# DYZhang09/ToC3D

Measured on AMD Instinct MI355X. Metric: multi-view frames/sec through ViT+ToC3D backbone, 6x(800x320), higher is better.
Workload: dtype bf16; 1 GPU; toc3d_faster EVA-02 ViT-L backbone + CPFPN neck, 6 views x 3x320x800 per frame, 1 frame per rank per step, random-init weights, prev_exists=True, injected Gumbel noise; frames_per_forward=1, launch=recorded launch plan replayed from C (toc3d_plan_run, HIP streams), view_groups=1, alias_outputs=True, gather_bytes=0

## Files before the change

include/toc3d.h:

```cpp
#ifndef TOC3D_H_
#define TOC3D_H_

#include <stdint.h>

#ifdef __cplusplus
extern "C" {
#endif

#define TOC3D_ABI_VERSION 10

#define TOC3D_OK 0
#define TOC3D_ERR_ARG (-1)
#define TOC3D_ERR_UNSUPPORTED (-2)
#define TOC3D_ERR_LAUNCH (-3)

#define TOC3D_DTYPE_F32 0
#define TOC3D_DTYPE_BF16 1
#define TOC3D_DTYPE_F32X3 2
#define TOC3D_DTYPE_F32X6 3
#define TOC3D_DTYPE_F32X3W 4
#define TOC3D_DTYPE_F32X3P 5
#define TOC3D_DTYPE_F32X3WO 6
#define TOC3D_DTYPE_F32X3WA 7

#define TOC3D_EPI_BIAS 0
#define TOC3D_EPI_RESIDUAL 1
#define TOC3D_EPI_SWIGLU 2
#define TOC3D_EPI_GELU 3
#define TOC3D_EPI_SWIGLU_STATS 4
#define TOC3D_EPI_RESIDUAL_LN 5
#define TOC3D_EPI_RESIDUAL_STATS 6
#define TOC3D_EPI_SWIGLU_STATS_LN 7
// ... 89 lines not shown
                               const int32_t* count, const int32_t* count_k, const int32_t* npad, const void* pad_rot, int64_t stride,
                               int64_t nwin, int64_t max_count, int64_t num_heads, const float* v_bias,
                               int64_t n_prefetch, const void* const* prefetch_ptrs, const int64_t* prefetch_bytes, int64_t prefetch_workgroups,
                               toc3d_stream_t stream);

int toc3d_gather_merge_ln(int dtype, const float* x, int64_t C, const int32_t* tok, const float* wgt, const int32_t* crow_tok,
                          const int32_t* rep_row, int64_t nW, int64_t N, int64_t k, int64_t rows, const float* gamma,
                          const float* beta, float eps, float* shortcut, void* a_out, int64_t lda, toc3d_stream_t stream);
int toc3d_gather_merge_ln_ex(int dtype, const float* x, int64_t C, const int32_t* tok, const float* wgt, const int32_t* crow_tok,
                             const int32_t* rep_row, int64_t nW, int64_t N, int64_t k, int64_t rows, const float* gamma,
                             const float* beta, float eps, float* shortcut, void* a_out, int64_t lda, int64_t kept_copy, toc3d_stream_t stream);
#define TOC3D_GATHER_SPLIT_COUNTER_BYTES 16384
int64_t toc3d_gather_merge_ln_scratch_bytes(int64_t nW, int64_t C);
int toc3d_gather_merge_ln_split(int dtype, const float* x, int64_t C, const int32_t* tok, const float* wgt, const int32_t* crow_tok,
                                const int32_t* rep_row, int64_t nW, int64_t N, int64_t k, int64_t rows, const float* gamma,
                                const float* beta, float eps, float* shortcut, void* a_out, int64_t lda, int64_t kept_copy,
                                void* scratch, int64_t scratch_bytes, int64_t split, toc3d_stream_t stream);
int toc3d_rebase_layernorm_rows(int dtype, float* slow, int64_t C, const int32_t* rep_index, const int32_t* tok, const float* wgt, int64_t N,
                                int64_t k, const float* rep_raw1, const float* rep_raw2, const float* gamma, const float* beta, float eps,
                                void* out, int64_t ldo, int64_t rows, toc3d_stream_t stream);
int toc3d_scatter_update(float* x, int64_t C, const int32_t* tok, const int32_t* prow, int64_t nW, int64_t N, int64_t k,
                         const float* slow_out, const float* rep_raw1, const float* rep_raw2, const float* rep_raw3, const float* rep_raw4,
                         toc3d_stream_t stream);

int64_t toc3d_motion_weights_floats(void);
int toc3d_pack_motion_weights(const float* qe0_w, const float* qe0_b, const float* qe2_w, const float* qe2_b,
                              const float* pe_red_w, const float* pe_red_b, const float* pe_gam_w, const float* pe_gam_b,
                              const float* pe_bet_w, const float* pe_bet_b, const float* q_red_w, const float* q_red_b,
                              const float* q_gam_w, const float* q_gam_b, const float* q_bet_w, const float* q_bet_b,
                              const float* te_w, const float* te_b, const float* te_ln_w, const float* te_ln_b,
                              const float* pc_range, const float* dimt3, const float* dimt1, float* out,
                              toc3d_stream_t stream);
int toc3d_motion_queries(const float* w, int64_t n_stages, int64_t w_stride, const float* queries, const float* ref_points,
                         const float* vel, const void* timestamp, int timestamp_is_f64, const float* ego_pose,
                         const float* ego_pose_inv, int64_t B, int64_t Q, float* out, toc3d_stream_t stream);
int toc3d_collapse_query_scorer(const float* mq, const float* w_in, const float* b_in, const float* w_agg, const float* b_agg,
                                int64_t B, int64_t Q, int64_t C, float scale, float* wc, float* bc, toc3d_stream_t stream);
int toc3d_score_tokens(const float* x, int64_t C, const float* mask, const float* wc, const float* bc, const float* gumbel,
                       int64_t V, int64_t T, int64_t views_per_frame, float* pred, float* score, float* mask_out,
                       toc3d_stream_t stream);

int toc3d_gumbel_noise(float* out, int64_t n, uint64_t seed, uint64_t* state, toc3d_stream_t stream);
int toc3d_gumbel_from_bits(const uint32_t* bits, int64_t n, float* out, toc3d_stream_t stream);

int toc3d_global_mean_half(int dtype, void* t, int64_t ld, int64_t V, int64_t T, int64_t C, toc3d_stream_t stream);
int toc3d_score_head(int dtype, const void* f, int64_t ld, int64_t kdim, const float* w, const float* b, const float* gumbel,
// ... 68 lines not shown
```

toc3d_amd/backbone.py:

```python
from __future__ import annotations

import math
from functools import partial
from typing import Dict

import torch
import torch.nn as nn

from . import gemm, lib
from .gemm import DEFAULT_PRECISION, round_up
from .plan import MODES, DerivedState, EagerExec, run_frame
from .synth import MOTION_DIM, QUERY_DIM, rope_tables


class ToC3DViTReturnType:

    def __init__(self, img_feats=None, token_masks=None, attn_scores=None, keep_idx=None, drop_idx=None,
                 aux_outputs: list = None) -> None:
        self.img_feats = img_feats
        self.token_masks = token_masks
        self.attn_scores = attn_scores
        self.keep_idx = keep_idx
        self.drop_idx = drop_idx
        self.aux_outputs = aux_outputs
# ... 92 lines not shown
            nn.init.constant_(m.bias, 0)
    elif isinstance(m, nn.LayerNorm):
        nn.init.constant_(m.bias, 0)
        nn.init.constant_(m.weight, 1.0)


def schedule_defaults(precision):
    bf16 = precision == "bf16"
    fast = precision in ("bf16", "fp32x3")
    return dict(
        x3_attention=precision == "fp32x3",
        x3_planes=precision == "fp32x3",
        carry_compact=fast,
        fold_ffn_ln=fast,
        fold_norm2=fast,
        gathered_residual=True,
        prefetch_weights=192 if bf16 else 0,
        attn_rot=fast,
        gather_split=False,
        side_lanes=True,
        big_windows_first=True,
        launch_mode="plan",
    )


class _BackboneBase(DerivedState, nn.Module):
    LN_EPS = 1e-6
    SCORER_LN_EPS = 1e-5

    def _setup_common(self, img_size, patch_size, in_chans, embed_dim, depth, num_heads, mlp_ratio, qkv_bias,
                      use_abs_pos, pt_hw_seq_len, window_size, global_window_size, global_attn_indexes,
                      pretrain_img_size, pretrain_use_cls_token, out_feature, precision, img_norm_cfg=None, pad_size_divisor=32, schedule=None):
        assert precision in ("bf16", "fp32", "fp32x3", "fp32x6"), precision
        self.img_norm_cfg = None
        if img_norm_cfg is not None:
            self.img_norm_cfg = dict(mean=torch.tensor(list(img_norm_cfg["mean"]), dtype=torch.float32),
                                     std=torch.tensor(list(img_norm_cfg["std"]), dtype=torch.float32),
                                     to_rgb=bool(img_norm_cfg.get("to_rgb", True)))
            assert self.img_norm_cfg["mean"].numel() == 3 and self.img_norm_cfg["std"].numel() == 3
        self.pad_size_divisor = int(pad_size_divisor)
        assert self.pad_size_divisor % patch_size == 0, "PadMultiViewImage divisor must be a multiple of the patch size"
        if embed_dim // num_heads != 64 or embed_dim % num_heads:
            raise NotImplementedError("the HIP attention kernel is built for head_dim 64 (EVA-02 L/B/tiny test config)")
        if embed_dim % 64 or embed_dim > 1024:
            raise NotImplementedError("embed_dim must be a multiple of 64 and <= 1024")
        self.precision = precision
# ... 3 lines not shown
        self.global_attn_indexes = tuple(global_attn_indexes)
        self.pretrain_use_cls_token = pretrain_use_cls_token
        self.hidden_dim = int(embed_dim * mlp_ratio)
        self.patch_embed = _PatchEmbed(in_chans, embed_dim, patch_size)
        if use_abs_pos:
            npatch = (pretrain_img_size // patch_size) ** 2
            self.pos_embed = nn.Parameter(torch.zeros(1, npatch + (1 if pretrain_use_cls_token else 0), embed_dim))
        else:
            self.pos_embed = None
        half = embed_dim // num_heads // 2
        self.rope_win = _Rope(window_size, half, pt_hw_seq_len)
        self.rope_glb = _Rope(img_size // patch_size, half, pt_hw_seq_len)
        if img_size // patch_size != global_window_size:
            raise NotImplementedError("global RoPE table side (img_size/patch) must equal global_window_size")
        self._out_features = [out_feature]
        self._out_feature_channels = {out_feature: embed_dim}
        self._out_feature_strides = {out_feature: patch_size}
        self._drop_derived()
        self._tuned: Dict[tuple, int] = {}
        self.autotune = True
        self.alias_outputs = False
        self.view_groups = 1
        sched = schedule_defaults(precision)
        unknown = set(schedule or {}) - set(sched)
        if unknown:
            raise TypeError(f"unknown schedule switches {sorted(unknown)}; known: {sorted(sched)}")
        sched.update(schedule or {})
        for k_, v_ in sched.items():
            setattr(self, k_, v_)
        assert self.launch_mode in MODES, self.launch_mode
        self._stream_pool = []

    _DERIVED = dict(_packed=None, _plans={}, _sk_ws={}, _sk_ws_old=[])
    _INSTANCE = dict(_stream_pool=[])

    def __getstate__(self):
        d = super().__getstate__()
        if d.get("_gumbel_rng") is not None:
            d["_gumbel_rng"] = d["_gumbel_rng"].detach().to("cpu").clone()
        return d

    def __setstate__(self, d):
        if "gumbel_seed" in d and "_gumbel_seed" not in d:
            d = dict(d)
            d["_gumbel_seed"] = d.pop("gumbel_seed")
        super().__setstate__(d)

    def _accelerated(self, i):
        return False

    @property
    def _dts(self):
        return gemm.dtypes(self.precision, self.x3_planes, self.x3_attention)

    _dt = property(lambda self: self._dts.act)
    _tdt = property(lambda self: self._dts.torch)
    _dt_gemm = property(lambda self: self._dts.gemm)
    _dt_rows = property(lambda self: self._dts.rows)
    _dt_attn = property(lambda self: self._dts.attn)
    _x3p = property(lambda self: self._dts.x3p)

    def _block_side(self, i):
        return self.global_window_size if i in self.global_attn_indexes else self.window_size

    @staticmethod
    def _f32(t):
        return t.detach().float().contiguous()

# ... 160 lines not shown
    def _stem_im2col(self, plan, img):
        s = lib.stream_ptr()
        V = plan["V"]
        H, W = plan["h"] * self.patch_size, plan["w"] * self.patch_size
        Kp = plan["col"].shape[1]
        if img.dtype == torch.uint8:
            n = self.img_norm_cfg
            lib.call("toc3d_im2col_patches_u8", self._dt, img, V, img.shape[1], img.shape[2], n["mean"], n["std"], int(n["to_rgb"]),
                     plan["col"], Kp, H, W, self.patch_size, s)
        else:
            lib.call("toc3d_im2col_patches", self._dt, img, plan["col"], Kp, V, self.in_chans, H, W, self.patch_size, s)

    def _stem_gemm(self, plan, P):
        C = self.embed_dim
        pos = P["pos"][(plan["h"], plan["w"])]
        self._linear(lib.EPI_RESIDUAL, plan["col"], P["w_patch"], P["b_patch"], plan["x"], plan["M"], C, plan["col"].shape[1],
                     residual=pos, ldr=C, residual_row_mod=plan["T"] if pos is not None else 0)

    def _ensure_pos(self, P, h, w, dev):
        if (h, w) not in P["pos"]:
            P["pos"][(h, w)] = self._pos_for(h, w, dev)

    def _run_frame(self, master, n_lanes, frame_fn, variant=None):
        run_frame(master.setdefault("launch", {}).setdefault(variant, {}), self.launch_mode, n_lanes, frame_fn, self._stream_pool)

    def _attention(self, P, i, *args):
        s = lib.stream_ptr()
        if not self.prefetch_weights:
            lib.call("toc3d_window_attention", *args, s)
            return
        lib.call("toc3d_window_attention_pf", *args, *self._prefetch_args(P, i), s)

    def _prefetch_args(self, P, i):
        bp = P["blocks"][i]
        ts = [bp["wproj"], bp["w12"], bp["w3"]] + ([P["blocks"][i + 1]["wqkv"]] if i + 1 < self.depth else [])
        if not self.prefetch_weights:
            ts = []
        return (len(ts), *lib.ptr_arrays(ts, min_len=1), self.prefetch_weights)

    def _qkv_attention(self, P, i, plan, M, rope_rc, arows, aslots, count_q, count_k, npad, pad, stride, nwin, max_count, v_bias):
        bp = P["blocks"][i]
        C, dt = self.embed_dim, self._dt
        if self._rot_ok(stride):
            self._linear(lib.EPI_QKV_ROPE, plan["a"], bp["wqkv"], bp["bqkv"], plan["qkv"], M, 3 * C, C,
                         rope=(rope_rc, bp["rope_tab"], bp["rope_side"], lib.ATTN_ROT_Q_SCALE), a_planes=self._x3p, o_planes=self._x3p)
            if self._x3p:
                lib.call("toc3d_window_attention_rot", lib.F32X3P, plan["qkv"], 3 * C, plan["att"], C, arows, aslots, count_q, count_k, npad, pad, stride, nwin, max_count,
# ... 3 lines not shown
                     self.num_heads, v_bias, *self._prefetch_args(P, i), lib.stream_ptr())
            return
        self._linear(lib.EPI_BIAS, plan["a"], bp["wqkv"], bp["bqkv"], plan["qkv"], M, 3 * C, C, a_planes=self._x3p)
        self._attention(P, i, self._dt_attn, plan["qkv"], 3 * C, plan["att"], C, arows, aslots, count_q, count_k, npad, pad,
                        stride, nwin, max_count, self.num_heads, bp["cos"], bp["sin"], bp["rope_side"], v_bias, 64 ** -0.5)

    def _rot_ok(self, stride):
        if not self.attn_rot:
            return False
        if self.precision == "bf16":
            return stride <= 416
        return self._x3p and stride <= 1024

    def _proj(self, bp, plan, rows, out, rep_out, rep_index, res=None, res_index=None):
        C = self.embed_dim
        res = out if res is None else res
        kw = dict(residual=res, ldr=C, rep_out=rep_out, rep_index=rep_index, residual_index=res_index, a_planes=self._x3p)
        if self.fold_norm2:
            self._linear(lib.EPI_RESIDUAL_STATS, plan["att"], bp["wproj"], bp["bproj"], out, rows, C, C, stats_out=(plan["stats2"], plan["stats2_cap"]),
                         out_act=plan["a"], ld_act=C, o_planes=self._x3p, **kw)
        else:
            self._linear(lib.EPI_RESIDUAL, plan["att"], bp["wproj"], bp["bproj"], out, rows, C, C, **kw)

    def _mlp(self, bp, plan, rows, res, rep_out, rep_index):
        s = lib.stream_ptr()
        C, Hd = self.embed_dim, self.hidden_dim
        Hp = plan["hid"].shape[1]
        dt = self._dt
        if self.fold_ffn_ln:
            st, cap = plan["stats"], plan["stats_cap"]
            if self.fold_norm2:
                self._linear(lib.EPI_SWIGLU_STATS_LN, plan["a"], bp["w12"], bp["c2_12"], plan["hid"], rows, 2 * Hp, C, n_valid=Hd, stats_out=(st, cap),
                             stats_in=(plan["stats2"], plan["stats2_cap"], C // 64), col_sums=bp["c1_12"], ln_n=C, ln_eps=self.LN_EPS,
                             a_planes=self._x3p, o_planes=self._x3p)
            else:
                lib.call("toc3d_layernorm_rows", dt, res, C, None, None, bp["ln2_w"], bp["ln2_b"], self.LN_EPS, plan["a"], C, rows, C, s)
                self._linear(lib.EPI_SWIGLU_STATS, plan["a"], bp["w12"], bp["b12"], plan["hid"], rows, 2 * Hp, C, n_valid=Hd, stats_out=(st, cap), o_planes=self._x3p)
            self._linear(lib.EPI_RESIDUAL_LN, plan["hid"], bp["w3"], bp["c2"], res, rows, C, Hp, residual=res, ldr=C, rep_out=rep_out, rep_index=rep_index,
                         stats_in=(st, cap, -(-2 * Hp // 128)), col_sums=bp["c1"], ln_n=Hd, ln_eps=self.LN_EPS, a_planes=self._x3p)
            return
        lib.call("toc3d_layernorm_rows", dt, res, C, None, None, bp["ln2_w"], bp["ln2_b"], self.LN_EPS, plan["a"], C, rows, C, s)
        self._linear(lib.EPI_SWIGLU, plan["a"], bp["w12"], bp["b12"], plan["hid"], rows, 2 * Hp, C, n_valid=Hd)
        lib.call("toc3d_layernorm_act", dt, plan["hid"], Hp, bp["lnf_w"], bp["lnf_b"], self.LN_EPS, plan["hln"], Hp, rows, Hd, s)
        self._linear(lib.EPI_RESIDUAL, plan["hln"], bp["w3"], bp["b3"], res, rows, C, Hp, residual=res, ldr=C, rep_out=rep_out, rep_index=rep_index)

    def _dense_block(self, i, plan, P):
        s = lib.stream_ptr()
        bp = P["blocks"][i]
        C, M, dt = self.embed_dim, plan["M"], self._dt
        x = plan["x"]
        dm = plan["dense"][self._block_side(i)]
        lib.call("toc3d_layernorm_rows", self._dt_rows, x, C, None, None, bp["ln1_w"], bp["ln1_b"], self.LN_EPS, plan["a"], C, M, C, s)
        self._qkv_attention(P, i, plan, M, dm.get("rc"), dm["rows"], dm["slots"], dm["count"], None, dm["npad"], None, dm["N"], dm["nW"], dm["max_count"], bp["v_bias"])
        self._proj(bp, plan, M, x, None, None)
        self._mlp(bp, plan, M, x, None, None)

    def _group_layout(self, V, B):
        G = max(1, int(self.view_groups))
        vpf = V // B
        if G > 1 and V % G == 0:
            Vg = V // G
            if Vg % vpf == 0:
                return [(g * Vg, Vg, g * (Vg // vpf), Vg // vpf) for g in range(G)]
            if vpf % Vg == 0:
                return [(g * Vg, Vg, (g * Vg) // vpf, 1) for g in range(G)]
        return [(0, V, 0, B)]

# ... 376 lines not shown
            self._join_side(ex, lane, side, plan)
            plan["side_L"] = None
        sel = plan["sel"][(st, self._block_side(i))]
        nW, N, k, rows = sel["nW"], sel["N"], sel["k"], sel["rows"]
        slow = plan["slow"]
        if carry_in:
            lib.call("toc3d_rebase_layernorm_rows", self._dt_rows, slow, C, sel["rep_index"], sel["tok"], sel["wgt"], N, k, plan["rep1"], plan["rep2"],
                     bp["ln1_w"], bp["ln1_b"], self.LN_EPS, plan["a"], C, rows, s)
        elif self.gather_split:
            lib.call("toc3d_gather_merge_ln_split", self._dt_rows, plan["x"], C, sel["tok"], sel["wgt"], sel["crow_tok"], sel["rep_row"], nW, N, k, rows,
                     bp["ln1_w"], bp["ln1_b"], self.LN_EPS, slow, plan["a"], C, 0 if self.gathered_residual else 1,
                     plan["gm_scratch"], plan["gm_scratch"].numel() * 4, int(self.gather_split) if self.gather_split is not True else 0, s)
        else:
            lib.call("toc3d_gather_merge_ln_ex", self._dt_rows, plan["x"], C, sel["tok"], sel["wgt"], sel["crow_tok"], sel["rep_row"], nW, N, k, rows,
                     bp["ln1_w"], bp["ln1_b"], self.LN_EPS, slow, plan["a"], C, 0 if self.gathered_residual else 1, s)
        rot = self._rot_ok(k + 1)
        self._qkv_attention(P, i, plan, rows, sel["crow_rc"], sel["arows"], sel["aslots"], sel["acount_q"], sel["acount_k"], None,
                            bp["pad_rot"] if rot else bp["pad_qkv"], k + 1, nW, sel["max_q"], None)
        ra, rb = (plan["rep3"], plan["rep4"]) if carry_in else (plan["rep1"], plan["rep2"])
        if self.gathered_residual and not carry_in:
            self._proj(bp, plan, rows, slow, ra, sel["rep_index"], res=plan["x"], res_index=sel["crow_tok"])
        else:
            self._proj(bp, plan, rows, slow, ra, sel["rep_index"])
        self._mlp(bp, plan, rows, slow, rb, sel["rep_index"])
        if not carry_out:
            lib.call("toc3d_scatter_update", plan["x"], C, sel["tok"], sel["prow"], nW, N, k, slow, plan["rep1"], plan["rep2"],
                     plan["rep3"] if carry_in else None, plan["rep4"] if carry_in else None, s)

    def _carries(self, i):
        return (self.carry_compact and i + 1 < self.depth and self._accelerated(i) and self._accelerated(i + 1)
                and (i + 1) not in self.pruning_loc and self._block_side(i) == self._block_side(i + 1))

    @torch.no_grad()
    def forward(self, x, temp_queries=None, prev_exists=None, temp_ref_points=None, temp_vel=None, temp_timestamp=None,
                temp_ego_pose=None, ego_pose_inv=None, *args, gumbel_noise=None, **kwargs):
        if "forced_scores" in kwargs:
            raise TypeError("forced_scores is a test instrument: wrap the model with toc3d_amd.testing.instrument(model)")
        x, H, W = self._check_input(x)
        if self._packed is None:
            self._packed = self._pack()
            self._plans = {}
        P = self._packed
        dev = x.device
        V = x.shape[0]
        prev = bool(prev_exists.bool().flatten()[0].item()) if isinstance(prev_exists, torch.Tensor) else bool(prev_exists)
        B = temp_queries.shape[0] if temp_queries is not None else 1
        assert V % B == 0
        ns = len(self.pruning_loc)
        key = (tuple(x.shape), x.dtype, B, self.view_groups)
        if key in self._plans:
# ... 103 lines not shown
```

toc3d_amd/csrc/gemm.hip:

```cpp
#include <cstdlib>

#include "gemm_kernels.h"

thread_local bool g_bad_variant = false;

namespace {

int launch_gemm(int is_bf16, int epi, int variant, const GemmArgs& a, hipStream_t s) {
    switch (epi) {
        case TOC3D_EPI_BIAS: case TOC3D_EPI_GELU: case TOC3D_EPI_CONV3X3: return toc3d_gemm_launch_plain(is_bf16, epi, variant, a, s);
        case TOC3D_EPI_RESIDUAL: case TOC3D_EPI_RESIDUAL_LN: case TOC3D_EPI_RESIDUAL_STATS: return toc3d_gemm_launch_residual(is_bf16, epi, variant, a, s);
        case TOC3D_EPI_SWIGLU: case TOC3D_EPI_SWIGLU_STATS: case TOC3D_EPI_SWIGLU_STATS_LN: return toc3d_gemm_launch_swiglu(is_bf16, epi, variant, a, s);
        case TOC3D_EPI_QKV_ROPE: return toc3d_gemm_launch_rope(is_bf16, epi, variant, a, s);
        default: return TOC3D_ERR_ARG;
    }
}

__global__ __launch_bounds__(256) void x3_planes_kernel(const float* src, int64_t ld_src, float* dst, int64_t ld_dst, int64_t rows, int gpr) {
    const int64_t grp = (int64_t)blockIdx.x * 32 + (threadIdx.x >> 3);
    if (grp >= rows * gpr) return;
    const int64_t row = grp / gpr;
    const int g = (int)(grp % gpr), q = threadIdx.x & 7;
    const f32x4 v = *reinterpret_cast<const f32x4*>(src + row * ld_src + g * 32 + q * 4);
    const float x[4] = {v[0], v[1], v[2], v[3]};
// ... 225 lines not shown
        TOC3D_REQUIRE(stats_in != stats_out, "toc3d_linear: stats_in and stats_out must be different buffers");
    }
    if (epilogue == TOC3D_EPI_RESIDUAL_STATS)
        TOC3D_REQUIRE(out_act && ld_act >= N && ((uintptr_t)out_act % 8) == 0 && ld_act % 4 == 0, "toc3d_linear: EPI_RESIDUAL_STATS needs out_act [M, ld_act >= N], 8-byte aligned rows");
    if (e_swiglu) {
        TOC3D_REQUIRE(bias && N % 32 == 0 && n_valid > 0 && n_valid <= N / 2, "toc3d_linear: swiglu needs bias, N%%32==0, n_valid");
        TOC3D_REQUIRE(ldo >= N / 2, "toc3d_linear: swiglu ldo < N/2");
    } else {
        TOC3D_REQUIRE(ldo >= N, "toc3d_linear: ldo < N");
    }
    TOC3D_REQUIRE(!residual_index || (e_residual && residual && residual_row_mod == 0), "toc3d_linear: residual_index needs a residual epilogue, a residual buffer and no row modulus");
    if (e_residual) {
        TOC3D_REQUIRE(!residual || ldr >= N, "toc3d_linear: ldr < N");
        TOC3D_REQUIRE(!rep_index || rep_out, "toc3d_linear: rep_index set without rep_out");
    }
    const int64_t osz = e_residual ? 4 : (dtype == TOC3D_BF16 ? 2 : 4);
    const bool vec = ldo % 4 == 0 && (uintptr_t)out % (4 * osz) == 0 && (!residual || (ldr % 4 == 0 && (uintptr_t)residual % 16 == 0)) &&
                     (!rep_out || (N % 4 == 0 && (uintptr_t)rep_out % 16 == 0));
    static const bool wide_ok = [] { const char* e = getenv("TOC3D_WIDE_STORES"); return !(e && e[0] == '0'); }();
    const bool vec8 = wide_ok && vec && dtype == TOC3D_BF16 && !e_residual && epilogue != TOC3D_EPI_CONV3X3 && ldo % 8 == 0 && (uintptr_t)out % 16 == 0;
    a = GemmArgs{A, lda, W, ldw, bias, out, ldo, residual, ldr, (int)residual_row_mod, residual_index, rep_out, rep_index,
               (int)M, (int)N, (int)K, (int)n_valid, 0, vec ? 1 : 0, vec8 ? 1 : 0,
               stats_out, (int)stats_out_cap, stats_in, (int)(stats_in_cap & 0xffffffff), (int)(stats_in_cap >> 32), col_sums, ln_n > 0 ? (float)(1.0 / (double)ln_n) : 0.f, ln_eps, out_act, ld_act,
               0, 0, nullptr, nullptr, nullptr, 0, 1.0f, planes_a, planes, planes_o, 0, nullptr, nullptr, dtype == TOC3D_F32X3 ? 1 : 0};
    if (planes) {
        TOC3D_REQUIRE(epilogue != TOC3D_EPI_CONV3X3 || !planes_a, "toc3d_linear: the 3x3 conv gathers f32 activations (A cannot be planes)");
        const void* act_copy = epilogue == TOC3D_EPI_CONV3X3 ? nullptr : out_act;
        TOC3D_REQUIRE((!planes_o || ((!e_swiglu || (ldo % 32 == 0 && (uintptr_t)out % 16 == 0)) && (!act_copy || (ld_act % 32 == 0 && (uintptr_t)act_copy % 16 == 0)))) &&
                      (!planes_a || lda % 32 == 0),
                      "toc3d_linear: rows of (hi, lo) planes are whole 32-element groups on 16-byte boundaries: lda, ldo (SwiGLU) and ld_act must be multiples of 32");
    }
    if (epilogue == TOC3D_EPI_CONV3X3) {
        a.conv_h = (int)(ld_act >> 32); a.conv_w = (int)(ld_act & 0xffffffff); a.zeros = out_act;
        TOC3D_REQUIRE(a.conv_h > 0 && a.conv_w > 0 && a.zeros && M % ((int64_t)a.conv_h * a.conv_w) == 0 && K == 9 * lda, "toc3d_linear: EPI_CONV3X3 goes through toc3d_conv3x3_nhwc");
        a.out_act = nullptr; a.ld_act = 0;
    }
    return TOC3D_OK;
}

static_assert(TOC3D_SPLITK_TICKET_BYTES % 256 == 0, "the partial tiles start on a 256-byte boundary");
int64_t toc3d_linear_splitk_workspace_bytes(int variant, int64_t M, int64_t N) {
    const int split = variant / 1000;
    const int dims = toc3d_gemm_splitk_tile_dims(variant % 1000);
    if (split < 2 || split > TOC3D_SPLITK_MAX || dims == 0 || M < 0 || N <= 0) return -1;
    const int64_t bm = dims >> 16, bn = dims & 0xffff, elems = bm * bn;
    const int64_t tiles = ((M + bm - 1) / bm) * ((N + bn - 1) / bn);
    if (tiles * 4 > TOC3D_SPLITK_TICKET_BYTES) return -1;
    return TOC3D_SPLITK_TICKET_BYTES + tiles * split * elems * 4;
}

// ... 189 lines not shown
```

toc3d_amd/csrc/gemm_kernels.h:

```cpp
#pragma once
#include "capi.h"
#include "common.h"

struct GemmArgs {
    const void* A; int64_t lda;
    const void* W; int64_t ldw;
    const float* bias;
    void* out; int64_t ldo;
    const float* res; int64_t ldr; int res_mod;
    const int32_t* res_index;
    float* rep_out; const int32_t* rep_index;
    int M, N, K, n_valid;
    int order;
    int vec;
    int vec8;
    float* stats; int stats_cap;
    const float* stats_in; int stats_in_cap;
    int stats_in_slots;
    const float* c1; float ln_inv_n, ln_eps;
    void* out_act; int64_t ld_act;
    int conv_h, conv_w; const void* zeros;
    const int32_t* rope_rc;
    const float* rope_tab;
    int rope_L; float rope_scale;
    int a_planes, w_planes, out_planes;
    int split; float* sk_slabs; unsigned* sk_tickets;
    int fast_silu;
};

extern thread_local bool g_bad_variant;

int toc3d_gemm_launch_plain(int is_bf16, int epi, int variant, const GemmArgs& a, hipStream_t s);
int toc3d_gemm_launch_residual(int is_bf16, int epi, int variant, const GemmArgs& a, hipStream_t s);
int toc3d_gemm_launch_swiglu(int is_bf16, int epi, int variant, const GemmArgs& a, hipStream_t s);
int toc3d_gemm_launch_rope(int is_bf16, int epi, int variant, const GemmArgs& a, hipStream_t s);
int toc3d_gemm_launch_x3(int epi, int variant, const GemmArgs& a, hipStream_t s);
int toc3d_gemm_launch_x6(int epi, int variant, const GemmArgs& a, hipStream_t s);
int toc3d_gemm_launch_splitk(int dtype, int epi, int variant, const GemmArgs& a, hipStream_t s);
int toc3d_gemm_splitk_tile_dims(int variant);

#ifdef TOC3D_GEMM_TRACE
__device__ unsigned long long* toc3d_trace_buf;
#define TOC3D_TRACE(slot)                                                                                                   \
    do {                                                                                                                    \
        if (threadIdx.x == 0 && toc3d_trace_buf) toc3d_trace_buf[(size_t)blockIdx.x * 4 + (slot)] = __builtin_amdgcn_s_memrealtime(); \
    } while (0)
#define TOC3D_TRACE_END()                                                                                                   \
    do {                                                                                                                    \
        asm volatile("s_waitcnt vmcnt(0)" ::: "memory");                                                                    \
        TOC3D_TRACE(2);                                                                                                     \
// ... 390 lines not shown
            if constexpr (PAIR_OK) {
                if (pair && (i & 1) && keep_row) {
#pragma unroll
                    for (int j = 0; j < NT; ++j)
                        if (nok[j] == 4) store_planes4(keep_row, col0 + j * 16 + g * 4, keep[j]);
                    keep_row = nullptr;
                }
            }
            continue;
        }
        float mu = 0.f, rs = 1.f;
        if (LN_IN && epi_is_residual(EPI)) { const f32x2 v = lnrow[i * 16 + r16]; mu = v[0]; rs = v[1]; }
        (void)mu; (void)rs;
        if (epi_is_residual(EPI)) {
            const int rr = a.res_mod > 0 ? row % a.res_mod : row;
            const float* resrow = a.res ? a.res + (int64_t)rr * a.ldr : nullptr;
            float* orow = reinterpret_cast<float*>(a.out) + (int64_t)row * a.ldo;
            if (a.res_index) {
                const int ti = a.res_index[row];
                resrow = ti >= 0 ? a.res + (int64_t)ti * a.ldr : orow;
            }
            float* reprow = nullptr;
            if (a.rep_index) { const int ri = a.rep_index[row]; if (ri >= 0) reprow = a.rep_out + (int64_t)ri * a.N; }
#pragma unroll
            for (int j = 0; j < NT; ++j) {
                if (nok[j] == 0) continue;
                const int col = col0 + j * 16 + g * 4;
                float raw[4];
#pragma unroll
                for (int r = 0; r < 4; ++r) {
                    if (LN_IN) raw[r] = rs * (acc[i][j][r] - mu * ccol[j][r]) + bcol[j][r];
                    else raw[r] = acc[i][j][r] + bcol[j][r];
                }
                float sum4[4] = {0.f, 0.f, 0.f, 0.f};
                if (a.vec && nok[j] == 4) {
                    f32x4 rv = resrow ? *reinterpret_cast<const f32x4*>(resrow + col) : f32x4{0.f, 0.f, 0.f, 0.f};
#pragma unroll
                    for (int r = 0; r < 4; ++r) sum4[r] = rv[r] + raw[r];
                    epi_store4(orow + col, sum4);
                    if (reprow) *reinterpret_cast<f32x4*>(reprow + col) = f32x4{raw[0], raw[1], raw[2], raw[3]};
                } else {
                    for (int r = 0; r < nok[j]; ++r) {
                        sum4[r] = (resrow ? resrow[col + r] : 0.f) + raw[r];
                        orow[col + r] = sum4[r];
                        if (reprow) reprow[col + r] = raw[r];
                    }
// ... 890 lines not shown
```

toc3d_amd/csrc/tokens.hip:

```cpp
#include "capi.h"
#include "common.h"

#ifndef TOC3D_ROW_BANDS
#define TOC3D_ROW_BANDS 5
#endif
#define TOC3D_ROW_BLOCK_IF(bit, b, n) ((TOC3D_ROW_BANDS >> (bit)) & 1 ? xcd_remap((int)(b), (int)(n)) : (int)(b))
#define TOC3D_ROW_BLOCK_OFF_IF(bit, b, off, n) ((TOC3D_ROW_BANDS >> (bit)) & 1 ? xcd_remap_off((int)(b), (int)(off), (int)(n)) : (int)(b) - (int)(off))

namespace {

constexpr float PAD_SCORE = -1.0e6f;

template <int MAXV>
TOC3D_DEV void wave_ln_stats(const f32x4 (&v)[MAXV], int nvec, int lane, int C, float eps, float& mean, float& rstd) {
    float s = 0.f;
#pragma unroll
    for (int i = 0; i < MAXV; ++i)
        if (lane + 64 * i < nvec) s += (v[i][0] + v[i][1]) + (v[i][2] + v[i][3]);
    mean = wave_sum(s) / (float)C;
    float q = 0.f;
#pragma unroll
    for (int i = 0; i < MAXV; ++i)
        if (lane + 64 * i < nvec) {
            const float d0 = v[i][0] - mean, d1 = v[i][1] - mean, d2 = v[i][2] - mean, d3 = v[i][3] - mean;
// ... 542 lines not shown
    if (id >= (int64_t)nW * N) return;
    const int win = (int)(id / N), p = (int)(id % N);
    const int dst = tok[id];
    if (dst < 0) return;
    const int nvec = C >> 2;
    float* xr = x + (int64_t)dst * C;
    if (p < k) {
        const float* s = slow_out + (int64_t)prow[id] * C;
        for (int vi = lane; vi < nvec; vi += 64) *reinterpret_cast<f32x4*>(xr + 4 * vi) = *reinterpret_cast<const f32x4*>(s + 4 * vi);
    } else {
        const float* a = r1 + (int64_t)win * C;
        const float* b = r2 + (int64_t)win * C;
        for (int vi = lane; vi < nvec; vi += 64) {
            f32x4 v = *reinterpret_cast<const f32x4*>(xr + 4 * vi);
            v = (v + *reinterpret_cast<const f32x4*>(a + 4 * vi)) + *reinterpret_cast<const f32x4*>(b + 4 * vi);
            if (r3) {
                v = (v + *reinterpret_cast<const f32x4*>(r3 + (int64_t)win * C + 4 * vi)) + *reinterpret_cast<const f32x4*>(r4 + (int64_t)win * C + 4 * vi);
            }
            *reinterpret_cast<f32x4*>(xr + 4 * vi) = v;
        }
    }
}

template <typename T, int MAXV>
__global__ __launch_bounds__(256) void ln_rebase_kernel(float* __restrict__ slow, int C, const int32_t* __restrict__ rep_index,
                                                        const int32_t* __restrict__ tok, const float* __restrict__ wgt, int N, int k,
                                                        const float* __restrict__ r1, const float* __restrict__ r2,
                                                        const float* __restrict__ gamma, const float* __restrict__ beta, float eps,
                                                        T* __restrict__ out, int64_t ldo, int M) {
    const int wave = threadIdx.x >> 6, lane = threadIdx.x & 63;
    const int row = TOC3D_ROW_BLOCK_IF(0, blockIdx.x, gridDim.x) * 4 + wave;
    if (row >= M) return;
    const int nvec = C >> 2;
    const int win = rep_index[row];
    float* xr = slow + (int64_t)row * C;
    f32x4 v[MAXV];
#pragma unroll
    for (int i = 0; i < MAXV; ++i) {
        const int vi = lane + 64 * i;
        v[i] = vi < nvec ? *reinterpret_cast<const f32x4*>(xr + 4 * vi) : f32x4{0.f, 0.f, 0.f, 0.f};
    }
    if (win >= 0) {
        float w = 0.f;
        for (int j = k + lane; j < N; j += 64)
            if (tok[(int64_t)win * N + j] >= 0) w += wgt[(int64_t)win * N + j];
        const float f = 1.0f - wave_sum(w);
// ... 242 lines not shown
    return TOC3D_OK;
}


int toc3d_gather_merge_ln(int dtype, const float* x, int64_t C, const int32_t* tok, const float* wgt, const int32_t* crow_tok,
                          const int32_t* rep_row, int64_t nW, int64_t N, int64_t k, int64_t rows, const float* gamma,
                          const float* beta, float eps, float* shortcut, void* a_out, int64_t lda, toc3d_stream_t stream) {
    return toc3d_gather_merge_ln_ex(dtype, x, C, tok, wgt, crow_tok, rep_row, nW, N, k, rows, gamma, beta, eps, shortcut, a_out, lda, 1, stream);
}

int toc3d_scatter_update(float* x, int64_t C, const int32_t* tok, const int32_t* prow, int64_t nW, int64_t N, int64_t k,
                         const float* slow_out, const float* rep_raw1, const float* rep_raw2, const float* rep_raw3, const float* rep_raw4,
                         toc3d_stream_t stream) {
    TOC3D_REQUIRE(x && tok && prow && slow_out && rep_raw1 && rep_raw2, "toc3d_scatter_update: null buffer");
    TOC3D_REQUIRE((rep_raw3 == nullptr) == (rep_raw4 == nullptr), "toc3d_scatter_update: rep_raw3 and rep_raw4 come as a pair");
    TOC3D_REQUIRE(C > 0 && C % 4 == 0 && k >= 0 && k < N, "toc3d_scatter_update: bad dims");
    if (nW <= 0 || N <= 0) return TOC3D_OK;
    dim3 grid((unsigned)((nW * N + 3) / 4));
    toc3d_launch(scatter_update_kernel, grid, dim3(256), 0, as_stream(stream), x, (int)C, tok, prow, (int)nW, (int)N, (int)k, slow_out, rep_raw1, rep_raw2, rep_raw3, rep_raw4);
    TOC3D_LAUNCH_CHECK("toc3d_scatter_update");
    return TOC3D_OK;
}

int toc3d_rebase_layernorm_rows(int dtype, float* slow, int64_t C, const int32_t* rep_index, const int32_t* tok, const float* wgt, int64_t N,
                                int64_t k, const float* rep_raw1, const float* rep_raw2, const float* gamma, const float* beta, float eps,
                                void* out, int64_t ldo, int64_t rows, toc3d_stream_t stream) {
    TOC3D_REQUIRE(slow && rep_index && tok && wgt && rep_raw1 && rep_raw2 && gamma && beta && out, "toc3d_rebase_layernorm_rows: null buffer");
    TOC3D_REQUIRE(C > 0 && C % 4 == 0 && C <= 2048 && ldo >= C && ldo % 4 == 0 && k >= 0 && k < N, "toc3d_rebase_layernorm_rows: bad dims");
    if (rows <= 0) return TOC3D_OK;
    dim3 grid((unsigned)((rows + 3) / 4)), block(256);
    hipStream_t s = as_stream(stream);
#define LNB(T, MV) toc3d_launch((ln_rebase_kernel<T, MV>), grid, block, 0, s, slow, (int)C, rep_index, tok, wgt, (int)N, (int)k, rep_raw1, rep_raw2, gamma, beta, eps, (T*)out, ldo, (int)rows)
    if (dtype == TOC3D_BF16) { if (C <= 1024) LNB(bf16_t, 4); else LNB(bf16_t, 8); }
    else if (dtype == TOC3D_F32) { if (C <= 1024) LNB(float, 4); else LNB(float, 8); }
    else if (dtype == TOC3D_F32X3P) {
        TOC3D_REQUIRE(planes_rows_ok(out, ldo), "toc3d_rebase_layernorm_rows: rows of (hi, lo) planes start on 128-byte boundaries (out aligned, ldo a multiple of 32)");
        if (C <= 1024) LNB(f32p_t, 4); else LNB(f32p_t, 8);
    }
    else { toc3d_set_error("toc3d_rebase_layernorm_rows: bad dtype"); return TOC3D_ERR_ARG; }
#undef LNB
    TOC3D_LAUNCH_CHECK("toc3d_rebase_layernorm_rows");
    return TOC3D_OK;
}

int toc3d_copy_bytes(void* dst, const void* src, int64_t nbytes, toc3d_stream_t stream) {
    TOC3D_REQUIRE(nbytes >= 0 && (nbytes == 0 || (dst && src)), "toc3d_copy_bytes: bad arguments");
// ... 39 lines not shown
```

toc3d_amd/gemm.py:

```python
from __future__ import annotations

from typing import NamedTuple

import torch

from . import lib

DEFAULT_PRECISION = "fp32x3"


def round_up(a: int, b: int) -> int:
    return (a + b - 1) // b * b


class Dtypes(NamedTuple):
    act: int
    torch: torch.dtype
    gemm: int
    rows: int
    attn: int
    x3p: bool


def attn_dtype(precision, x3_attention, planes_out):
# ... 83 lines not shown
            e0.record()
            call(v, o, rep_s)
            e1.record()
            e1.synchronize()
            ts.append(e0.elapsed_time(e1))
        return min(ts)
    short = sorted((cold_time(v, 3), v) for v in cands)[:4]
    return min((cold_time(v, 9), v) for _, v in short)[1]


def _splitk_workspace(owner, need, device, stream):
    pool = owner.__dict__.setdefault("_sk_ws", {})
    key = (device.index, stream)
    ws = pool.get(key)
    if ws is None or ws.numel() * 4 < need:
        if ws is not None:
            owner.__dict__.setdefault("_sk_ws_old", []).append(ws)
        ws = pool[key] = torch.zeros((need + 3) // 4, dtype=torch.int32, device=device)
    return ws


def linear(owner, epi, A, W, bias, out, M, N, K, *, lda=None, ldw=None, ldo=None, residual=None, ldr=0, residual_row_mod=0, rep_out=None, rep_index=None,
           n_valid=0, stats_out=(None, 0), stats_in=(None, 0, 0), col_sums=None, ln_n=0, ln_eps=0.0, out_act=None, ld_act=0, residual_index=None,
           conv=None, rope=None, a_planes=False, o_planes=False, variant=None):
    dtg = launch_dtype(dtypes_of(owner).gemm, a_planes, o_planes, rope=epi == lib.EPI_QKV_ROPE)
    lda, ldw, ldo = (A.shape[1] if lda is None else lda), (W.shape[1] if ldw is None else ldw), (out.shape[1] if ldo is None else ldo)
    s = lib.stream_ptr()
    var = owner._tuned.get((epi, M, N, K)) if variant is None else variant
    if epi == lib.EPI_QKV_ROPE:
        if var is None:
            var = owner._tuned.get((lib.EPI_BIAS, M, N, K), 0)
        lib.call("toc3d_linear_qkv_rope", dtg, var, A, lda, W, ldw, bias, out, ldo, M, N, K, *rope, s)
        return
    if conv is not None:
        out_act, ld_act = conv[0], (conv[1] << 32) | conv[2]

    def args(v, o, rep):
        return (dtg, epi, v, A, lda, W, ldw, bias, o, ldo, residual, ldr, residual_row_mod, rep, rep_index, M, N, K, n_valid,
                stats_out[0], stats_out[1], stats_in[0], stats_in[1] | stats_in[2] << 32, col_sums, ln_n, ln_eps, out_act, ld_act, residual_index)
    if var is None:
        var = 0
        if lib.recording():
            lib.call("toc3d_linear_fused", *args(0, out, rep_out), s)
            return
        if owner.autotune and not torch.cuda.is_current_stream_capturing():
            var = _tune(dtg, epi, lambda v, o, rep: lib.call("toc3d_linear_fused", *args(v, o, rep), s), out, ldo, rep_out, M)
        owner._tuned[(epi, M, N, K)] = var
    if var >= 1000:
        ws = _splitk_workspace(owner, int(lib.load().toc3d_linear_splitk_workspace_bytes(var, M, N)), out.device, s)
        lib.call("toc3d_linear_fused_ws", *args(var, out, rep_out), ws, ws.numel() * 4, s)
        return
    lib.call("toc3d_linear_fused", *args(var, out, rep_out), s)
```

toc3d_amd/lib.py:

```python
from __future__ import annotations

import ctypes
import os
import re
import threading

_HERE = os.path.dirname(os.path.abspath(__file__))
LIB_PATH = os.path.join(_HERE, os.environ.get("TOC3D_LIB", "libtoc3d_gfx950.so"))
HEADER_PATH = os.path.join(os.path.dirname(_HERE), "include", "toc3d.h")

ABI_VERSION = 10
F32, BF16, F32X3, F32X6, F32X3W, F32X3P, F32X3WO, F32X3WA = 0, 1, 2, 3, 4, 5, 6, 7
EPI_BIAS, EPI_RESIDUAL, EPI_SWIGLU, EPI_GELU, EPI_SWIGLU_STATS, EPI_RESIDUAL_LN, EPI_RESIDUAL_STATS, EPI_SWIGLU_STATS_LN, EPI_CONV3X3, EPI_QKV_ROPE = 0, 1, 2, 3, 4, 5, 6, 7, 8, 9
ATTN_ROT_Q_SCALE = 64 ** -0.5 * 1.4426950408889634
NO_FUSED = (None, 0, None, 0, None, 0, 0.0, None, 0, None)
PRODUCT_VARIANTS = (1, 8, 9, 10, 13, 14, 15, 16, 17, 19, 22, 24, 26, 27, 28, 29, 30, 33, 45, 47, 49, 51, 52, 53, 54, 55, 56, 57, 58, 59, 60, 61, 62, 63, 64, 65, 66)
X3_PLANES_ONLY_VARIANTS = (54, 55, 56, 57, 58, 59, 60, 61, 62, 63)


def has_variant(v: int) -> bool:
    return (v % 100) in PRODUCT_VARIANTS

_P, _I64, _I, _F = ctypes.c_void_p, ctypes.c_int64, ctypes.c_int, ctypes.c_float

_SIGS = {
    "toc3d_linear": "iiplplpplpllppllllp",
    "toc3d_linear_ex": "iiiplplpplpllppllllp",
    "toc3d_linear_fused": "iiiplplpplpllppllll" + "plplplf" + "pl" + "p" + "p",
    "toc3d_linear_fused_ws": "iiiplplpplpllppllll" + "plplplf" + "pl" + "p" + "pl" + "p",
    "toc3d_pack_swiglu_lnfold": "ippppppllpppllp",
    "toc3d_pack_weight_lnfold": "ippppllpllppp",
    "toc3d_conv3x3_nhwc": "iiplplpplllllpp",
    "toc3d_pack_weight": "ipllpllp",
    "toc3d_x3_planes": "plplllp",
    "toc3d_pack_swiglu": "ippppllppllp",
    "toc3d_im2col_patches": "ippllllllp",
    "toc3d_normalize_images": "plllppipllp",
    "toc3d_im2col_patches_u8": "iplllppipllllp",
    "toc3d_abs_pos_bicubic": "pllpllp",
    "toc3d_layernorm_rows": "iplppppfplllp",
    "toc3d_layernorm_act": "iplppfplllp",
    "toc3d_window_map_dense": "llllppppp",
    "toc3d_window_attention": "iplplppppppllllpplpfp",
    "toc3d_window_attention_pf": "iplplppppppllllpplpf" + "lppl" + "p",
    "toc3d_rank_desc": "pllpp",
    "toc3d_window_topk": "plllllppppppppppppp",
    "toc3d_linear_qkv_rope": "iiplplppllllpplfp",
    "toc3d_window_attention_rot": "iplplppppppllllp" + "lppl" + "p",
    "toc3d_gather_merge_ln": "iplppppllllppfpplp",
    "toc3d_gather_merge_ln_ex": "iplppppllllppfppllp",
    "toc3d_gather_merge_ln_split": "iplppppllllppfppll" + "pll" + "p",
    "toc3d_scatter_update": "plpplllpppppp",
    "toc3d_rebase_layernorm_rows": "iplpppllppppfpllp",
    "toc3d_pack_motion_weights": "p" * 24 + "p",
    "toc3d_motion_queries": "pllppppippllpp",
    "toc3d_collapse_query_scorer": "ppppplllfppp",
    "toc3d_score_tokens": "plpppplllpppp",
    "toc3d_gumbel_noise": "plLpp",
    "toc3d_gumbel_from_bits": "plpp",
    "toc3d_global_mean_half": "ipllllp",
    "toc3d_score_head": "ipllppplpppp",
    "toc3d_nhwc_to_nchw": "pplllp",
    "toc3d_im2col_3x3": "ipplllllp",
    "toc3d_head_frustum_inputs": "ippppllllllllplplpp",
    "toc3d_relu_inplace": "iplp",
    "toc3d_nchw_to_rows": "ippllllp",
    "toc3d_mln_apply": "ipppllpplp",
    "toc3d_se_gate": "ppplp",
    "toc3d_memory_pre_update": "pppppppppplllllip",
    "toc3d_memory_scores": "pllpp",
    "toc3d_memory_post_update": "ppppppppppppplpppllllllp",
    "toc3d_mha_attention": "iplplplpllllllfp",
    "toc3d_mha_attention_ex": "iplplplplplplllllllfp",
    "toc3d_add_layernorm_pos": "iplppfplplplplppplllp",
    "toc3d_add_pos_rows": "iplplplplllp",
# ... 123 lines not shown
```

Before: 209.4 frames/s.

## Write MLP output rows directly into scattered token positions, scatter only dropped tokens

The final MLP GEMM epilogue can now write each compact output row straight into its destination row of the full token tensor through an out_index array, carried in the stats_out slot. A new scatter_update_dropped kernel then only adds the representative residual deltas to dropped tokens, so kept tokens are no longer written out and re-copied by the full scatter pass. The path is controlled by a new schedule switch that follows fold_ffn_ln, which makes it on by default for bf16, and the cached launch plan is rebuilt when the switch changes. The cost is an extra indexed store path in the GEMM epilogue and more validation logic around the reused stats argument.

Result: no change. 210.4 frames/s (median of 6 runs) (+0.5%).

```diff
diff --git a/include/toc3d.h b/include/toc3d.h
--- a/include/toc3d.h
+++ b/include/toc3d.h
@@ -7,7 +7,7 @@
 extern "C" {
 #endif
 
-#define TOC3D_ABI_VERSION 10
+#define TOC3D_ABI_VERSION 11
 
 #define TOC3D_OK 0
 #define TOC3D_ERR_ARG (-1)
@@ -143,6 +143,8 @@
 int toc3d_scatter_update(float* x, int64_t C, const int32_t* tok, const int32_t* prow, int64_t nW, int64_t N, int64_t k,
                          const float* slow_out, const float* rep_raw1, const float* rep_raw2, const float* rep_raw3, const float* rep_raw4,
                          toc3d_stream_t stream);
+int toc3d_scatter_update_dropped(float* x, int64_t C, const int32_t* tok, const int32_t* prow, int64_t nW, int64_t N, int64_t k,
+                                 const float* rep_raw1, const float* rep_raw2, const float* rep_raw3, const float* rep_raw4, toc3d_stream_t stream);
 
 int64_t toc3d_motion_weights_floats(void);
 int toc3d_pack_motion_weights(const float* qe0_w, const float* qe0_b, const float* qe2_w, const float* qe2_b,
diff --git a/toc3d_amd/backbone.py b/toc3d_amd/backbone.py
--- a/toc3d_amd/backbone.py
+++ b/toc3d_amd/backbone.py
@@ -138,6 +138,11 @@
         big_windows_first=True,
         launch_mode="plan",
     )
+
+
+SCHEDULE_FOLLOWERS = dict(
+    scattered_output="fold_ffn_ln",
+)
 
 
 class _BackboneBase(DerivedState, nn.Module):
@@ -187,10 +192,12 @@
         self.alias_outputs = False
         self.view_groups = 1
         sched = schedule_defaults(precision)
-        unknown = set(schedule or {}) - set(sched)
+        unknown = set(schedule or {}) - set(sched) - set(SCHEDULE_FOLLOWERS)
         if unknown:
-            raise TypeError(f"unknown schedule switches {sorted(unknown)}; known: {sorted(sched)}")
+            raise TypeError(f"unknown schedule switches {sorted(unknown)}; known: {sorted(set(sched) | set(SCHEDULE_FOLLOWERS))}")
         sched.update(schedule or {})
+        for k_, leader in SCHEDULE_FOLLOWERS.items():
+            sched.setdefault(k_, bool(sched[leader]))
         for k_, v_ in sched.items():
             setattr(self, k_, v_)
         assert self.launch_mode in MODES, self.launch_mode
@@ -209,6 +216,9 @@
         if "gumbel_seed" in d and "_gumbel_seed" not in d:
             d = dict(d)
             d["_gumbel_seed"] = d.pop("gumbel_seed")
+        missing = {k_: bool(d[leader]) for k_, leader in SCHEDULE_FOLLOWERS.items() if k_ not in d and leader in d}
+        if missing:
+            d = {**d, **missing}
         super().__setstate__(d)
 
     def _accelerated(self, i):
@@ -415,7 +425,12 @@
             P["pos"][(h, w)] = self._pos_for(h, w, dev)
 
     def _run_frame(self, master, n_lanes, frame_fn, variant=None):
-        run_frame(master.setdefault("launch", {}).setdefault(variant, {}), self.launch_mode, n_lanes, frame_fn, self._stream_pool)
+        state = master.setdefault("launch", {}).setdefault(variant, {})
+        sig = tuple(bool(getattr(self, k_, False)) for k_ in SCHEDULE_FOLLOWERS)
+        if state.setdefault("followers", sig) != sig:
+            state.pop("cplan", None)
+            state["followers"] = sig
+        run_frame(state, self.launch_mode, n_lanes, frame_fn, self._stream_pool)
 
     def _attention(self, P, i, *args):
         s = lib.stream_ptr()
@@ -465,7 +480,7 @@
         else:
             self._linear(lib.EPI_RESIDUAL, plan["att"], bp["wproj"], bp["bproj"], out, rows, C, C, **kw)
 
-    def _mlp(self, bp, plan, rows, res, rep_out, rep_index):
+    def _mlp(self, bp, plan, rows, res, rep_out, rep_index, out_x=None, out_index=None):
         s = lib.stream_ptr()
         C, Hd = self.embed_dim, self.hidden_dim
         Hp = plan["hid"].shape[1]
@@ -480,12 +495,14 @@
                 lib.call("toc3d_layernorm_rows", dt, res, C, None, None, bp["ln2_w"], bp["ln2_b"], self.LN_EPS, plan["a"], C, rows, C, s)
                 self._linear(lib.EPI_SWIGLU_STATS, plan["a"], bp["w12"], bp["b12"], plan["hid"], rows, 2 * Hp, C, n_valid=Hd, stats_out=(st, cap), o_planes=self._x3p)
             self._linear(lib.EPI_RESIDUAL_LN, plan["hid"], bp["w3"], bp["c2"], res, rows, C, Hp, residual=res, ldr=C, rep_out=rep_out, rep_index=rep_index,
-                         stats_in=(st, cap, -(-2 * Hp // 128)), col_sums=bp["c1"], ln_n=Hd, ln_eps=self.LN_EPS, a_planes=self._x3p)
+                         stats_in=(st, cap, -(-2 * Hp // 128)), col_sums=bp["c1"], ln_n=Hd, ln_eps=self.LN_EPS, a_planes=self._x3p,
+                         **(dict(out_act=out_x, ld_act=C, out_index=out_index) if out_index is not None else {}))
             return
         lib.call("toc3d_layernorm_rows", dt, res, C, None, None, bp["ln2_w"], bp["ln2_b"], self.LN_EPS, plan["a"], C, rows, C, s)
         self._linear(lib.EPI_SWIGLU, plan["a"], bp["w12"], bp["b12"], plan["hid"], rows, 2 * Hp, C, n_valid=Hd)
         lib.call("toc3d_layernorm_act", dt, plan["hid"], Hp, bp["lnf_w"], bp["lnf_b"], self.LN_EPS, plan["hln"], Hp, rows, Hd, s)
-        self._linear(lib.EPI_RESIDUAL, plan["hln"], bp["w3"], bp["b3"], res, rows, C, Hp, residual=res, ldr=C, rep_out=rep_out, rep_index=rep_index)
+        self._linear(lib.EPI_RESIDUAL, plan["hln"], bp["w3"], bp["b3"], res, rows, C, Hp, residual=res, ldr=C, rep_out=rep_out, rep_index=rep_index,
+                     **(dict(out_act=out_x, ld_act=C, out_index=out_index) if out_index is not None else {}))
 
     def _dense_block(self, i, plan, P):
         s = lib.stream_ptr()
@@ -908,10 +925,16 @@
             self._proj(bp, plan, rows, slow, ra, sel["rep_index"], res=plan["x"], res_index=sel["crow_tok"])
         else:
             self._proj(bp, plan, rows, slow, ra, sel["rep_index"])
-        self._mlp(bp, plan, rows, slow, rb, sel["rep_index"])
-        if not carry_out:
-            lib.call("toc3d_scatter_update", plan["x"], C, sel["tok"], sel["prow"], nW, N, k, slow, plan["rep1"], plan["rep2"],
-                     plan["rep3"] if carry_in else None, plan["rep4"] if carry_in else None, s)
+        if carry_out:
+            self._mlp(bp, plan, rows, slow, rb, sel["rep_index"])
+            return
+        r34 = (plan["rep3"], plan["rep4"]) if carry_in else (None, None)
+        if self.scattered_output:
+            self._mlp(bp, plan, rows, slow, rb, sel["rep_index"], out_x=plan["x"], out_index=sel["crow_tok"])
+            lib.call("toc3d_scatter_update_dropped", plan["x"], C, sel["tok"], sel["prow"], nW, N, k, plan["rep1"], plan["rep2"], *r34, s)
+        else:
+            self._mlp(bp, plan, rows, slow, rb, sel["rep_index"])
+            lib.call("toc3d_scatter_update", plan["x"], C, sel["tok"], sel["prow"], nW, N, k, slow, plan["rep1"], plan["rep2"], *r34, s)
 
     def _carries(self, i):
         return (self.carry_compact and i + 1 < self.depth and self._accelerated(i) and self._accelerated(i + 1)
diff --git a/toc3d_amd/csrc/gemm.hip b/toc3d_amd/csrc/gemm.hip
--- a/toc3d_amd/csrc/gemm.hip
+++ b/toc3d_amd/csrc/gemm.hip
@@ -271,10 +271,18 @@
     a = GemmArgs{A, lda, W, ldw, bias, out, ldo, residual, ldr, (int)residual_row_mod, residual_index, rep_out, rep_index,
                (int)M, (int)N, (int)K, (int)n_valid, 0, vec ? 1 : 0, vec8 ? 1 : 0,
                stats_out, (int)stats_out_cap, stats_in, (int)(stats_in_cap & 0xffffffff), (int)(stats_in_cap >> 32), col_sums, ln_n > 0 ? (float)(1.0 / (double)ln_n) : 0.f, ln_eps, out_act, ld_act,
-               0, 0, nullptr, nullptr, nullptr, 0, 1.0f, planes_a, planes, planes_o, 0, nullptr, nullptr, dtype == TOC3D_F32X3 ? 1 : 0};
+               0, 0, nullptr, nullptr, nullptr, 0, 1.0f, planes_a, planes, planes_o, 0, nullptr, nullptr, dtype == TOC3D_F32X3 ? 1 : 0, nullptr};
+    const bool scattered = (epilogue == TOC3D_EPI_RESIDUAL || epilogue == TOC3D_EPI_RESIDUAL_LN) && out_act;
+    if (scattered) {
+        TOC3D_REQUIRE(stats_out && stats_out_cap == 0 && ((uintptr_t)stats_out % 4) == 0,
+                      "toc3d_linear: epilogue %d with out_act (scattered output rows) takes the int32 row index [M] in stats_out, with stats_out_cap = 0", epilogue);
+        TOC3D_REQUIRE(ld_act >= N && ld_act % 4 == 0 && ((uintptr_t)out_act % 16) == 0, "toc3d_linear: scattered output rows need out_act f32 [*, ld_act >= N], 16-byte aligned rows");
+        a.out_index = reinterpret_cast<const int32_t*>(stats_out);
+        a.stats = nullptr; a.stats_cap = 0;
+    }
     if (planes) {
         TOC3D_REQUIRE(epilogue != TOC3D_EPI_CONV3X3 || !planes_a, "toc3d_linear: the 3x3 conv gathers f32 activations (A cannot be planes)");
-        const void* act_copy = epilogue == TOC3D_EPI_CONV3X3 ? nullptr : out_act;
+        const void* act_copy = (epilogue == TOC3D_EPI_CONV3X3 || scattered) ? nullptr : out_act;
         TOC3D_REQUIRE((!planes_o || ((!e_swiglu || (ldo % 32 == 0 && (uintptr_t)out % 16 == 0)) && (!act_copy || (ld_act % 32 == 0 && (uintptr_t)act_copy % 16 == 0)))) &&
                       (!planes_a || lda % 32 == 0),
                       "toc3d_linear: rows of (hi, lo) planes are whole 32-element groups on 16-byte boundaries: lda, ldo (SwiGLU) and ld_act must be multiples of 32");
diff --git a/toc3d_amd/csrc/gemm_kernels.h b/toc3d_amd/csrc/gemm_kernels.h
--- a/toc3d_amd/csrc/gemm_kernels.h
+++ b/toc3d_amd/csrc/gemm_kernels.h
@@ -26,6 +26,7 @@
     int a_planes, w_planes, out_planes;
     int split; float* sk_slabs; unsigned* sk_tickets;
     int fast_silu;
+    const int32_t* out_index;
 };
 
 extern thread_local bool g_bad_variant;
@@ -462,6 +463,9 @@
             }
             float* reprow = nullptr;
             if (a.rep_index) { const int ri = a.rep_index[row]; if (ri >= 0) reprow = a.rep_out + (int64_t)ri * a.N; }
+            if constexpr (EPI == TOC3D_EPI_RESIDUAL || EPI == TOC3D_EPI_RESIDUAL_LN) {
+                if (a.out_index) { const int oi = a.out_index[row]; if (oi >= 0) orow = reinterpret_cast<float*>(a.out_act) + (int64_t)oi * a.ld_act; }
+            }
 #pragma unroll
             for (int j = 0; j < NT; ++j) {
                 if (nok[j] == 0) continue;
diff --git a/toc3d_amd/csrc/tokens.hip b/toc3d_amd/csrc/tokens.hip
--- a/toc3d_amd/csrc/tokens.hip
+++ b/toc3d_amd/csrc/tokens.hip
@@ -588,6 +588,30 @@
     }
 }
 
+__global__ __launch_bounds__(256) void scatter_update_dropped_kernel(float* __restrict__ x, int C, const int32_t* __restrict__ tok, int nW, int N, int k,
+                                                                     const float* __restrict__ r1, const float* __restrict__ r2,
+                                                                     const float* __restrict__ r3, const float* __restrict__ r4) {
+    const int wave = threadIdx.x >> 6, lane = threadIdx.x & 63;
+    const int D = N - k;
+    const int64_t id = (int64_t)TOC3D_ROW_BLOCK_IF(2, blockIdx.x, gridDim.x) * 4 + wave;
+    if (id >= (int64_t)nW * D) return;
+    const int win = (int)(id / D), p = k + (int)(id % D);
+    const int dst = tok[(int64_t)win * N + p];
+    if (dst < 0) return;
+    const int nvec = C >> 2;
+    float* xr = x + (int64_t)dst * C;
+    const float* a = r1 + (int64_t)win * C;
+    const float* b = r2 + (int64_t)win * C;
+    for (int vi = lane; vi < nvec; vi += 64) {
+        f32x4 v = *reinterpret_cast<const f32x4*>(xr + 4 * vi);
+        v = (v + *reinterpret_cast<const f32x4*>(a + 4 * vi)) + *reinterpret_cast<const f32x4*>(b + 4 * vi);
+        if (r3) {
+            v = (v + *reinterpret_cast<const f32x4*>(r3 + (int64_t)win * C + 4 * vi)) + *reinterpret_cast<const f32x4*>(r4 + (int64_t)win * C + 4 * vi);
+        }
+        *reinterpret_cast<f32x4*>(xr + 4 * vi) = v;
+    }
+}
+
 template <typename T, int MAXV>
 __global__ __launch_bounds__(256) void ln_rebase_kernel(float* __restrict__ slow, int C, const int32_t* __restrict__ rep_index,
                                                         const int32_t* __restrict__ tok, const float* __restrict__ wgt, int N, int k,
@@ -876,6 +900,20 @@
     return TOC3D_OK;
 }
 
+int toc3d_scatter_update_dropped(float* x, int64_t C, const int32_t* tok, const int32_t* prow, int64_t nW, int64_t N, int64_t k,
+                                 const float* rep_raw1, const float* rep_raw2, const float* rep_raw3, const float* rep_raw4, toc3d_stream_t stream) {
+    (void)prow;
+    TOC3D_REQUIRE(x && tok && rep_raw1 && rep_raw2, "toc3d_scatter_update_dropped: null buffer");
+    TOC3D_REQUIRE((rep_raw3 == nullptr) == (rep_raw4 == nullptr), "toc3d_scatter_update_dropped: rep_raw3 and rep_raw4 come as a pair");
+    TOC3D_REQUIRE(C > 0 && C % 4 == 0 && k >= 0 && k < N, "toc3d_scatter_update_dropped: bad dims");
+    TOC3D_REQUIRE(nW <= 0 || nW * (N - k) < ((int64_t)1 << 31), "toc3d_scatter_update_dropped: too many slots");
+    if (nW <= 0) return TOC3D_OK;
+    dim3 grid((unsigned)((nW * (N - k) + 3) / 4));
+    toc3d_launch(scatter_update_dropped_kernel, grid, dim3(256), 0, as_stream(stream), x, (int)C, tok, (int)nW, (int)N, (int)k, rep_raw1, rep_raw2, rep_raw3, rep_raw4);
+    TOC3D_LAUNCH_CHECK("toc3d_scatter_update_dropped");
+    return TOC3D_OK;
+}
+
 int toc3d_rebase_layernorm_rows(int dtype, float* slow, int64_t C, const int32_t* rep_index, const int32_t* tok, const float* wgt, int64_t N,
                                 int64_t k, const float* rep_raw1, const float* rep_raw2, const float* gamma, const float* beta, float eps,
                                 void* out, int64_t ldo, int64_t rows, toc3d_stream_t stream) {
diff --git a/toc3d_amd/gemm.py b/toc3d_amd/gemm.py
--- a/toc3d_amd/gemm.py
+++ b/toc3d_amd/gemm.py
@@ -129,7 +129,7 @@
 
 def linear(owner, epi, A, W, bias, out, M, N, K, *, lda=None, ldw=None, ldo=None, residual=None, ldr=0, residual_row_mod=0, rep_out=None, rep_index=None,
            n_valid=0, stats_out=(None, 0), stats_in=(None, 0, 0), col_sums=None, ln_n=0, ln_eps=0.0, out_act=None, ld_act=0, residual_index=None,
-           conv=None, rope=None, a_planes=False, o_planes=False, variant=None):
+           out_index=None, conv=None, rope=None, a_planes=False, o_planes=False, variant=None):
     dtg = launch_dtype(dtypes_of(owner).gemm, a_planes, o_planes, rope=epi == lib.EPI_QKV_ROPE)
     lda, ldw, ldo = (A.shape[1] if lda is None else lda), (W.shape[1] if ldw is None else ldw), (out.shape[1] if ldo is None else ldo)
     s = lib.stream_ptr()
@@ -141,6 +141,9 @@
         return
     if conv is not None:
         out_act, ld_act = conv[0], (conv[1] << 32) | conv[2]
+    if out_index is not None:
+        assert epi in (lib.EPI_RESIDUAL, lib.EPI_RESIDUAL_LN) and out_act is not None and stats_out[0] is None, "scattered output rows: a residual epilogue without statistics"
+        stats_out = (out_index, 0)
 
     def args(v, o, rep):
         return (dtg, epi, v, A, lda, W, ldw, bias, o, ldo, residual, ldr, residual_row_mod, rep, rep_index, M, N, K, n_valid,
diff --git a/toc3d_amd/lib.py b/toc3d_amd/lib.py
--- a/toc3d_amd/lib.py
+++ b/toc3d_amd/lib.py
@@ -9,7 +9,7 @@
 LIB_PATH = os.path.join(_HERE, os.environ.get("TOC3D_LIB", "libtoc3d_gfx950.so"))
 HEADER_PATH = os.path.join(os.path.dirname(_HERE), "include", "toc3d.h")
 
-ABI_VERSION = 10
+ABI_VERSION = 11
 F32, BF16, F32X3, F32X6, F32X3W, F32X3P, F32X3WO, F32X3WA = 0, 1, 2, 3, 4, 5, 6, 7
 EPI_BIAS, EPI_RESIDUAL, EPI_SWIGLU, EPI_GELU, EPI_SWIGLU_STATS, EPI_RESIDUAL_LN, EPI_RESIDUAL_STATS, EPI_SWIGLU_STATS_LN, EPI_CONV3X3, EPI_QKV_ROPE = 0, 1, 2, 3, 4, 5, 6, 7, 8, 9
 ATTN_ROT_Q_SCALE = 64 ** -0.5 * 1.4426950408889634
@@ -51,6 +51,7 @@
     "toc3d_gather_merge_ln_ex": "iplppppllllppfppllp",
     "toc3d_gather_merge_ln_split": "iplppppllllppfppll" + "pll" + "p",
     "toc3d_scatter_update": "plpplllpppppp",
+    "toc3d_scatter_update_dropped": "plpplllppppp",
     "toc3d_rebase_layernorm_rows": "iplpppllppppfpllp",
     "toc3d_pack_motion_weights": "p" * 24 + "p",
     "toc3d_motion_queries": "pllppppippllpp",
```
